# CESSProject/DeOSS

Measured on AMD Instinct MI355X. Metric: device-resident GiB/s hashed to Merkle root; 1/2/4/8 MI355X scaling, higher is better.
Workload: dtype u32; 1 GPU; BASELINE configs[1]: 1 object of 8 GiB (8589934592 B) in 1 chunk-range shard(s) of 8 GiB, chunk 33554432 B (256 leaves); object_bytes=8589934592, chunk=33554432, leaves=256, parallelism=single GPU

## Files before the change

deoss_amd/csrc/merkle_kernels.hpp:

```cpp
#pragma once
#include "sha256_gfx950.hpp"

namespace dm {

constexpr int kBlock = 256;
constexpr int kLeafFuseMax = 8;
constexpr int kReduceTile = 512;

struct LeafArgs {
    const uint8_t* base;
    uint64_t pitch;
    uint64_t leaf_len;
    uint64_t last_len;
    const uint64_t* addrs;
    const uint64_t* lens;
    uint64_t nleaves;
    uint64_t byte_off;
    uint64_t byte_end;
    uint32_t* state;
    uint8_t* digests;
    uint8_t* level_out;
    uint32_t fuse_levels;
};

__device__ __forceinline__ void load_digest(const uint8_t* p, uint32_t (&v)[8]) {
    const uint4* q = reinterpret_cast<const uint4*>(p);
    uint4 x = q[0], y = q[1];
    v[0] = bswap32(x.x); v[1] = bswap32(x.y); v[2] = bswap32(x.z); v[3] = bswap32(x.w);
    v[4] = bswap32(y.x); v[5] = bswap32(y.y); v[6] = bswap32(y.z); v[7] = bswap32(y.w);
}

__device__ __forceinline__ void store_digest(uint8_t* p, const uint32_t (&v)[8]) {
    uint4* q = reinterpret_cast<uint4*>(p);
    q[0] = make_uint4(bswap32(v[0]), bswap32(v[1]), bswap32(v[2]), bswap32(v[3]));
    q[1] = make_uint4(bswap32(v[4]), bswap32(v[5]), bswap32(v[6]), bswap32(v[7]));
}


typedef uint32_t u32x4_t __attribute__((ext_vector_type(4)));
typedef __attribute__((address_space(1))) const u32x4_t global_u32x4;

typedef __attribute__((address_space(1))) const uint8_t global_u8;
typedef __attribute__((address_space(1))) const uint32_t global_u32;

struct Blk { u32x4_t q0, q1, q2, q3; };
__device__ __forceinline__ const global_u8* gbytes(const uint8_t* p) { return (const global_u8*)p; }

template <bool ALIGNED>
__device__ __forceinline__ Blk load_block(const uint8_t* p) {
    Blk b;
    if constexpr (ALIGNED) {
        const global_u32x4* q = (const global_u32x4*)(p);
        b.q0 = q[0]; b.q1 = q[1]; b.q2 = q[2]; b.q3 = q[3];
    } else {
        uint8_t t[64];
        const global_u8* g = gbytes(p);
#pragma unroll
        for (int k = 0; k < 64; k++) t[k] = g[k];
        __builtin_memcpy(&b, t, 64);
    }
    return b;
}

__device__ __forceinline__ void block_words(const Blk& b, uint32_t (&w)[16]) {
    w[0] = bswap32(b.q0.x);  w[1] = bswap32(b.q0.y);  w[2] = bswap32(b.q0.z);  w[3] = bswap32(b.q0.w);
    w[4] = bswap32(b.q1.x);  w[5] = bswap32(b.q1.y);  w[6] = bswap32(b.q1.z);  w[7] = bswap32(b.q1.w);
    w[8] = bswap32(b.q2.x);  w[9] = bswap32(b.q2.y);  w[10] = bswap32(b.q2.z); w[11] = bswap32(b.q2.w);
    w[12] = bswap32(b.q3.x); w[13] = bswap32(b.q3.y); w[14] = bswap32(b.q3.z); w[15] = bswap32(b.q3.w);
}

#ifndef DM_K1_LINES
#define DM_K1_LINES 1
#endif
template <bool ALIGNED>
__device__ __forceinline__ void absorb_blocks(uint32_t (&st)[8], const uint8_t* p, uint64_t nb) {
    if (nb == 0) return;
    if constexpr (ALIGNED && DM_K1_LINES) {
        const uint64_t last = nb - 1;
        Blk c0 = load_block<true>(p), c1 = load_block<true>(p + 64 * (last < 1 ? last : 1));
        for (uint64_t b = 0; b < nb; b += 2) {
            const uint64_t b2 = b + 2 < last ? b + 2 : last, b3 = b + 3 < last ? b + 3 : last;
            const Blk n0 = load_block<true>(p + 64 * b2), n1 = load_block<true>(p + 64 * b3);
            __builtin_amdgcn_sched_barrier(0);
            uint32_t w[16];
            block_words(c0, w);
            compress(st, w);
            if (b + 1 < nb) {
                block_words(c1, w);
                compress(st, w);
            }
            c0 = n0;
            c1 = n1;
        }
        return;
    }
    Blk cur = load_block<ALIGNED>(p);
    for (uint64_t b = 0; b < nb; b++) {
        uint32_t w[16];
        block_words(cur, w);
        if (b + 1 < nb) cur = load_block<ALIGNED>(p + 64 * (b + 1));
        compress(st, w);
    }
}

template <bool ALIGNED>
__device__ __forceinline__ void absorb_tail(uint32_t (&st)[8], const uint8_t* p, uint32_t r, uint64_t len) {
    uint32_t w[16];
#pragma unroll
    for (int k = 0; k < 16; k++) {
        uint32_t v = 0;
        if ((uint32_t)(4 * k + 4) <= r) {
            if constexpr (ALIGNED) {
                v = bswap32(*(const global_u32*)(p + 4 * k));
            } else {
                const global_u8* g = gbytes(p);
                v = ((uint32_t)g[4 * k] << 24) | ((uint32_t)g[4 * k + 1] << 16) |
                    ((uint32_t)g[4 * k + 2] << 8) | (uint32_t)g[4 * k + 3];
            }
        } else if ((uint32_t)(4 * k) <= r) {
#pragma unroll
            for (int j = 0; j < 4; j++) {
                uint32_t idx = 4 * k + j;
                uint32_t byte = idx < r ? (uint32_t)gbytes(p)[idx] : (idx == r ? 0x80u : 0u);
                v |= byte << (24 - 8 * j);
            }
        }
        w[k] = v;
    }
    const uint64_t bits = len * 8;
    if (r <= 55) {
        w[14] = (uint32_t)(bits >> 32);
        w[15] = (uint32_t)bits;
        compress(st, w);
    } else {
        compress(st, w);
#pragma unroll
        for (int k = 0; k < 14; k++) w[k] = 0;
        w[14] = (uint32_t)(bits >> 32);
        w[15] = (uint32_t)bits;
        compress(st, w);
    }
}

__device__ __forceinline__ uint32_t lds_reduce(uint32_t (*a)[8], uint32_t (*b)[8], uint32_t cnt,
                                               uint32_t levels, uint32_t (**res)[8]) {
    const uint32_t t = threadIdx.x;
    for (uint32_t l = 0; l < levels; l++) {
        const uint32_t next = (cnt + 1) >> 1;
        if (t < next) {
            uint32_t L[8], R[8], o[8];
            const uint32_t ri = (2 * t + 1 < cnt) ? 2 * t + 1 : cnt - 1;
#pragma unroll
            for (int k = 0; k < 8; k++) { L[k] = a[2 * t][k]; R[k] = a[ri][k]; }
            node_hash(L, R, o);
#pragma unroll
            for (int k = 0; k < 8; k++) b[t][k] = o[k];
        }
        __syncthreads();
        uint32_t (*tmp)[8] = a; a = b; b = tmp;
        cnt = next;
    }
    *res = a;
    return cnt;
}

struct LeafView {
    const uint8_t* p;
    uint64_t len;
    uint64_t have;
    uint64_t nb;
    bool fin;
    bool active;
};

template <bool TABLE>
__device__ __forceinline__ LeafView leaf_view(const LeafArgs& a, uint64_t i) {
    LeafView v{};
    v.active = i < a.nleaves;
    if (!v.active) {
        v.p = a.base;
        return v;
    }
    if constexpr (TABLE) {
        v.p = reinterpret_cast<const uint8_t*>(a.addrs[i]);
        v.len = a.lens[i];
    } else {
        v.p = a.base + i * a.pitch;
        v.len = (i + 1 == a.nleaves) ? a.last_len : a.leaf_len;
    }
    const uint64_t b0 = a.byte_off;
    const uint64_t end = v.len < a.byte_end ? v.len : a.byte_end;
    v.have = end > b0 ? end - b0 : 0;
    v.fin = (b0 < v.len && v.len <= a.byte_end) || (v.len == 0 && b0 == 0);
    v.nb = v.have / 64;
    return v;
}

__device__ __forceinline__ void load_or_init_state(const LeafArgs& a, uint64_t i, uint32_t (&st)[8]) {
    if (a.state != nullptr && a.byte_off != 0) {
#pragma unroll
        for (int k = 0; k < 8; k++) st[k] = a.state[i * 8 + k];
    } else {
        init_state(st);
    }
}

template <bool ALIGNED>
__device__ __forceinline__ void leaf_epilogue(const LeafArgs& a, uint64_t i, const LeafView& v, uint32_t (&st)[8]) {
    if (v.fin) {
        absorb_tail<ALIGNED>(st, v.p + 64 * v.nb, (uint32_t)(v.have - 64 * v.nb), v.len);
        if (a.digests != nullptr) store_digest(a.digests + 32 * i, st);
    } else if (a.state != nullptr && v.have != 0) {
#pragma unroll
        for (int k = 0; k < 8; k++) a.state[i * 8 + k] = st[k];
    }
}

__device__ __forceinline__ uint64_t wave_min_u64(uint64_t x) {
#pragma unroll
    for (int o = 32; o > 0; o >>= 1) {
        const uint64_t y = __shfl_xor(x, o, 64);
        x = y < x ? y : x;
    }
    return x;
}

__device__ __forceinline__ uint64_t uniform_u64(uint64_t x) {
    return ((uint64_t)__builtin_amdgcn_readfirstlane((uint32_t)(x >> 32)) << 32) |
           __builtin_amdgcn_readfirstlane((uint32_t)x);
}

__device__ __forceinline__ uint64_t wave_max_u64(uint64_t x) {
#pragma unroll
    for (int o = 32; o > 0; o >>= 1) {
        const uint64_t y = __shfl_xor(x, o, 64);
        x = y > x ? y : x;
    }
    return x;
}

template <bool TABLE, bool ALIGNED>
__global__ __launch_bounds__(kBlock) void leaf_kernel(LeafArgs a) {
    __shared__ uint32_t lds_a[kBlock][8];
    __shared__ uint32_t lds_b[kBlock / 2][8];
    const uint64_t i = (uint64_t)blockIdx.x * kBlock + threadIdx.x;
    const LeafView v = leaf_view<TABLE>(a, i);
    const bool active = v.active;
    uint32_t st[8];
    if (active) {
        load_or_init_state(a, i, st);
        absorb_blocks<ALIGNED>(st, v.p, v.nb);
        leaf_epilogue<ALIGNED>(a, i, v, st);
    }
    if (a.fuse_levels == 0) return;
    const uint64_t first = (uint64_t)blockIdx.x * kBlock;
    const uint32_t cnt = (uint32_t)((a.nleaves - first) < kBlock ? (a.nleaves - first) : kBlock);
    if (active) {
#pragma unroll
        for (int k = 0; k < 8; k++) lds_a[threadIdx.x][k] = st[k];
    }
    __syncthreads();
    uint32_t (*res)[8];
    const uint32_t out_cnt = lds_reduce(lds_a, lds_b, cnt, a.fuse_levels, &res);
    if (threadIdx.x < out_cnt) {
        uint32_t v[8];
#pragma unroll
        for (int k = 0; k < 8; k++) v[k] = res[threadIdx.x][k];
        const uint64_t o = (uint64_t)blockIdx.x * (kBlock >> a.fuse_levels) + threadIdx.x;
        store_digest(a.level_out + 32 * o, v);
    }
}

constexpr int kLatLeaves = 64;
constexpr int kLatThreads = 128;
constexpr int kLatRing = 2;
constexpr int kLatFuseMax = 6;

__device__ __forceinline__ void rounds_from_kw(uint32_t (&st)[8], const uint4 (*kw)[kLatLeaves], uint32_t lane) {
    uint32_t a = st[0], b = st[1], c = st[2], d = st[3], e = st[4], f = st[5], g = st[6], h = st[7];
    uint4 x = kw[0][lane], y = kw[1][lane];
#pragma unroll
    for (int q = 0; q < 16; q += 2) {
        uint4 nx = x, ny = y;
        if (q + 2 < 16) {
            nx = kw[q + 2][lane];
            ny = kw[q + 3][lane];
        }
        DM_SHA_ROUND(a, b, c, d, e, f, g, h, x.x);
        DM_SHA_ROUND(h, a, b, c, d, e, f, g, x.y);
        DM_SHA_ROUND(g, h, a, b, c, d, e, f, x.z);
        DM_SHA_ROUND(f, g, h, a, b, c, d, e, x.w);
        DM_SHA_ROUND(e, f, g, h, a, b, c, d, y.x);
        DM_SHA_ROUND(d, e, f, g, h, a, b, c, y.y);
        DM_SHA_ROUND(c, d, e, f, g, h, a, b, y.z);
        DM_SHA_ROUND(b, c, d, e, f, g, h, a, y.w);
        x = nx;
        y = ny;
    }
    st[0] += a; st[1] += b; st[2] += c; st[3] += d;
    st[4] += e; st[5] += f; st[6] += g; st[7] += h;
}

__device__ __forceinline__ void schedule_to_lds(uint32_t (&w)[16], uint4 (*kw)[kLatLeaves], uint32_t lane) {
// ... 88 lines not shown
        X7 = t_ + dpp_swap_pairs(y_);                                                  \
    } while (0)

__device__ __forceinline__ void pair_rounds_from_kw(uint32_t (&x)[4], const uint4 (*kw)[kLatLeaves], uint32_t lane,
                                                    uint32_t sh1, uint32_t sh2, uint32_t sh3, uint32_t msk,
                                                    bool lane_b) {
    uint32_t x4 = x[0], x5 = x[1], x6 = x[2], x7 = x[3];
    uint4 q = kw[0][lane];
#pragma unroll
    for (int g = 0; g < 16; g++) {
        uint4 nq = q;
        if (g + 1 < 16) nq = kw[g + 1][lane];
        DM_PAIR_ROUND(x4, x5, x6, x7, q.x);
        DM_PAIR_ROUND(x7, x4, x5, x6, q.y);
        DM_PAIR_ROUND(x6, x7, x4, x5, q.z);
        DM_PAIR_ROUND(x5, x6, x7, x4, q.w);
        q = nq;
    }
    x[0] += x4; x[1] += x5; x[2] += x6; x[3] += x7;
}

template <bool TABLE, bool ALIGNED>
__global__ __launch_bounds__(kLatThreads) void leaf_kernel_pair(LeafArgs a) {
    __shared__ uint4 ring[kLatRing][16][kLatLeaves];
    __shared__ uint32_t lds_a[kPairLeaves][8];
    __shared__ uint32_t lds_b[kPairLeaves / 2][8];
    const uint32_t lane = threadIdx.x & (kLatLeaves - 1);
    const bool producer = __builtin_amdgcn_readfirstlane(threadIdx.x) < kLatLeaves;
    const bool lane_b = (lane & 1) != 0;
    const uint32_t c = lane >> 1;
    const uint64_t first = (uint64_t)blockIdx.x * kPairLeaves;
    const uint64_t i = first + c;
    const LeafView v = leaf_view<TABLE>(a, i);
    const uint64_t NB = wave_max_u64(v.nb);
    if (producer) {
        Blk cur;
        if (v.nb > 0 && !lane_b) cur = load_block<ALIGNED>(v.p);
        for (uint64_t b = 0; b < NB; b++) {
            if (b < v.nb) {
                uint32_t w[16];
                block_words(cur, w);
                if (b + 1 < v.nb && !lane_b) cur = load_block<ALIGNED>(v.p + 64 * (b + 1));
                uint4 (*kw)[kLatLeaves] = ring[b % kLatRing];
#pragma unroll
                for (int q = 0; q < 16; q++) {
                    uint32_t u[4];
#pragma unroll
                    for (int j = 0; j < 4; j++) {
                        const int t = 4 * q + j;
                        uint32_t wt;
                        if (t < 16) {
                            wt = w[t];
                        } else {
                            wt = ssig1(w[(t - 2) & 15]) + w[(t - 7) & 15] + ssig0(w[(t - 15) & 15]) + w[t & 15];
                            w[t & 15] = wt;
                        }
                        u[j] = lane_b ? 0u : kSha256K[t] + wt;
                    }
                    kw[q][lane] = make_uint4(u[0], u[1], u[2], u[3]);
                }
            }
            __syncthreads();
        }
        __syncthreads();
    } else {
        const uint32_t sh1 = lane_b ? 2 : 6, sh2 = lane_b ? 13 : 11, sh3 = lane_b ? 22 : 25;
        const uint32_t msk = lane_b ? 0u : ~0u;
        uint32_t st0[8];
        if (v.active) load_or_init_state(a, i, st0);
        else init_state(st0);
        uint32_t x[4];
#pragma unroll
        for (int k = 0; k < 4; k++) x[k] = lane_b ? st0[k] : st0[4 + k];
        __syncthreads();
        for (uint64_t b = 0; b < NB; b++) {
            if (b < v.nb) pair_rounds_from_kw(x, ring[b % kLatRing], lane, sh1, sh2, sh3, msk, lane_b);
            __syncthreads();
        }
        uint32_t st[8];
#pragma unroll
        for (int k = 0; k < 4; k++) {
            const uint32_t other = dpp_swap_pairs(x[k]);
            st[k] = lane_b ? x[k] : other;
            st[4 + k] = lane_b ? other : x[k];
        }
        if (v.active && !lane_b) {
            leaf_epilogue<ALIGNED>(a, i, v, st);
#pragma unroll
            for (int k = 0; k < 8; k++) lds_a[c][k] = st[k];
        }
    }
    if (a.fuse_levels == 0) return;
    __syncthreads();
    const uint32_t cnt = (uint32_t)((a.nleaves - first) < kPairLeaves ? (a.nleaves - first) : kPairLeaves);
    uint32_t (*res)[8];
    const uint32_t out_cnt = lds_reduce(lds_a, lds_b, cnt, a.fuse_levels, &res);
    if (threadIdx.x < out_cnt) {
        uint32_t o8[8];
#pragma unroll
        for (int k = 0; k < 8; k++) o8[k] = res[threadIdx.x][k];
        const uint64_t o = (uint64_t)blockIdx.x * (kPairLeaves >> a.fuse_levels) + threadIdx.x;
        store_digest(a.level_out + 32 * o, o8);
    }
}

constexpr int kQuadLeaves = 8;
constexpr int kQuadBlocks = 8;
constexpr int kQuadFuseMax = 3;
constexpr int kQuadRow = kQuadLeaves;
constexpr size_t kQuadLdsBytes = sizeof(uint4) * kLatRing * 16 * kQuadBlocks * kQuadRow + 4 * 8 * kQuadLeaves +
                                 4 * 8 * (kQuadLeaves / 2);
static_assert(4 * kQuadLdsBytes <= (160u << 10), "four compact K1Q workgroups must fit a CU's LDS");

#define DM_QS_HEAD(X4, X5, X6)                                                                   \
    "v_alignbit_b32 %[r], %[" X4 "], %[" X4 "], %[sh]\n\t"                                      \
    "v_bitop3_b32 %[f], %[" X4 "], %[" X5 "], %[msk] bitop3:0x1e\n\t"                          \
    "v_bitop3_b32 %[f], %[f], %[" X6 "], %[" X5 "] bitop3:0xca\n\t"                             \
    "v_xor_b32_dpp %[s], %[r], %[r] quad_perm:[1,2,0,3] row_mask:0xf bank_mask:0xf\n\t"
#define DM_QS_SIGMA "v_xor_b32_dpp %[s], %[r], %[s] quad_perm:[2,0,1,3] row_mask:0xf bank_mask:0xf\n\t"
#define DM_QS_STEP_Q(X4, X5, X6, X7, H, HN, VN, QP)                                             \
    DM_QS_HEAD(X4, X5, X6)                                                                       \
    "v_sub_u32_dpp %[" X6 "], %[" VN "], %[" X6 "] quad_perm:" QP " row_mask:0xf bank_mask:0x3\n\t" \
    DM_QS_SIGMA                                                                                  \
    "v_sub_u32_dpp %[" HN "], %[" X4 "], %[" X6 "] row_ror:8 row_mask:0xf bank_mask:0xf\n\t"    \
    "v_add3_u32 %[" X7 "], %[s], %[f], %[" H "]\n\t"
#define DM_QS_STEP(X4, X5, X6, X7, H, HN, VN) DM_QS_STEP_Q(X4, X5, X6, X7, H, HN, VN, "[0,1,2,3]")
#define DM_QS_STEP_A(X4, X5, X6, X7, H, HN)                                                     \
    DM_QS_HEAD(X4, X5, X6)                                                                       \
    DM_QS_SIGMA                                                                                  \
    "v_sub_u32_dpp %[" HN "], %[" X4 "], %[" X6 "] row_ror:8 row_mask:0xf bank_mask:0xf\n\t"    \
    "v_add3_u32 %[" X7 "], %[s], %[f], %[" H "]\n\t"
#define DM_QS_STEP_END(X4, X5, X6, X7, H)                                                       \
    DM_QS_HEAD(X4, X5, X6)                                                                       \
    DM_QS_SIGMA                                                                                  \
    "v_add3_u32 %[" X7 "], %[s], %[f], %[" H "]\n\t"
#define DM_QS_STEPS4V(V0, V1, V2, V3)                                                          \
    DM_QS_STEP("a", "b", "c", "d", "h", "g", V0) DM_QS_STEP("d", "a", "b", "c", "g", "h", V1)   \
    DM_QS_STEP("c", "d", "a", "b", "h", "g", V2) DM_QS_STEP("b", "c", "d", "a", "g", "h", V3)
#define DM_QS_ALIGN_MIS ".p2align 3\n\t.if %[mis]\n\ts_nop 0\n\t.endif\n\t"
#define DM_QS_PROLOGUE(V) DM_QS_PROLOGUE_AT(V, DM_QS_ALIGN_MIS, "[0,1,2,3]")
#define DM_QS_PROLOGUE_AT(V, ALIGN, QP)                                                           \
    "s_nop 1\n\t" ALIGN                                                                          \
    "v_sub_u32_dpp %[d], %[" V "], %[d] quad_perm:" QP " row_mask:0xf bank_mask:0x3\n\t"         \
    "v_sub_u32_dpp %[h], %[b], %[d] row_ror:8 row_mask:0xf bank_mask:0xf\n\t"
#define DM_QS_RESTORE_A(P, X) "v_mov_b32_dpp %[" P "], %[" X "] quad_perm:[0,1,2,3] row_mask:0xf bank_mask:0xc\n\t"
#define DM_QS_GROUP0(V0, V1, V2, V3)                                                             \
    DM_QS_STEP("a", "b", "c", "d", "h", "g", V0) DM_QS_RESTORE_A("d", "x3")                      \
    DM_QS_STEP("d", "a", "b", "c", "g", "h", V1) DM_QS_RESTORE_A("c", "x2")                      \
    DM_QS_STEP("c", "d", "a", "b", "h", "g", V2) DM_QS_STEP("b", "c", "d", "a", "g", "h", V3)
#define DM_QS_FF(X, P, BANKS) "v_add_u32_dpp %[" X "], %[" P "], %[" X "] quad_perm:[0,1,2,3] row_mask:0xf bank_mask:" BANKS "\n\t"
#define DM_QS_TAIL(V0, V1, V2)                                                                   \
    DM_QS_STEP("a", "b", "c", "d", "h", "g", V0) DM_QS_STEP("d", "a", "b", "c", "g", "h", V1)   \
    DM_QS_STEP("c", "d", "a", "b", "h", "g", V2) DM_QS_STEP_A("b", "c", "d", "a", "g", "h")      \
    DM_QS_FF("x3", "d", "0x3") DM_QS_FF("x2", "c", "0x3") DM_QS_FF("x1", "b", "0x3")             \
    DM_QS_FF("x0", "a", "0x3")                                                                   \
    DM_QS_STEP_A("a", "b", "c", "d", "h", "g") DM_QS_STEP_END("d", "a", "b", "c", "g")           \
    DM_QS_FF("x0", "a", "0xc") DM_QS_FF("x1", "b", "0xc") DM_QS_FF("x3", "d", "0xc")             \
    DM_QS_FF("x2", "c", "0xc")
#define DM_QS_STEPS4Q(V0, Q0, V1, Q1, V2, Q2, V3, Q3)                                          \
    DM_QS_STEP_Q("a", "b", "c", "d", "h", "g", V0, Q0) DM_QS_STEP_Q("d", "a", "b", "c", "g", "h", V1, Q1) \
    DM_QS_STEP_Q("c", "d", "a", "b", "h", "g", V2, Q2) DM_QS_STEP_Q("b", "c", "d", "a", "g", "h", V3, Q3)
#define DM_QS_GROUP0Q(V0, Q0, V1, Q1, V2, Q2, V3, Q3)                                          \
    DM_QS_STEP_Q("a", "b", "c", "d", "h", "g", V0, Q0) DM_QS_RESTORE_A("d", "x3")              \
    DM_QS_STEP_Q("d", "a", "b", "c", "g", "h", V1, Q1) DM_QS_RESTORE_A("c", "x2")              \
    DM_QS_STEP_Q("c", "d", "a", "b", "h", "g", V2, Q2) DM_QS_STEP_Q("b", "c", "d", "a", "g", "h", V3, Q3)
#define DM_QS_TAILQ(V0, Q0, V1, Q1, V2, Q2)                                                     \
    DM_QS_STEP_Q("a", "b", "c", "d", "h", "g", V0, Q0) DM_QS_STEP_Q("d", "a", "b", "c", "g", "h", V1, Q1) \
    DM_QS_STEP_Q("c", "d", "a", "b", "h", "g", V2, Q2) DM_QS_STEP_A("b", "c", "d", "a", "g", "h") \
    DM_QS_FF("x3", "d", "0x3") DM_QS_FF("x2", "c", "0x3") DM_QS_FF("x1", "b", "0x3")             \
    DM_QS_FF("x0", "a", "0x3")                                                                   \
    DM_QS_STEP_A("a", "b", "c", "d", "h", "g") DM_QS_STEP_END("d", "a", "b", "c", "g")           \
    DM_QS_FF("x0", "a", "0xc") DM_QS_FF("x1", "b", "0xc") DM_QS_FF("x3", "d", "0xc")             \
    DM_QS_FF("x2", "c", "0xc")
#define DM_QS_OUT                                                                                \
    : [a] "+v"(p0), [b] "+v"(p1), [c] "+v"(p2), [d] "+v"(p3), [h] "+v"(h), [g] "+v"(g),           \
      [x0] "+v"(x[0]), [x1] "+v"(x[1]), [x2] "+v"(x[2]), [x3] "+v"(x[3]), [r] "=&v"(r_),          \
      [f] "=&v"(f_), [s] "=&v"(s_)
#define DM_QS_OPS DM_QS_OUT : [mis] "i"(MIS ? 1 : 0), [sh] "v"(sh.x), [msk] "v"(msk), [v0] "v"(v0), [v1] "v"(v1), [v2] "v"(v2), [v3] "v"(v3)

template <bool MIS, class KW>
__device__ __forceinline__ void quad_block_skewed(uint32_t (&x)[4], KW kw, uint3 sh, uint32_t msk) {
    uint32_t p0 = x[0], p1 = x[1], p2 = x[2], p3 = x[3], h = 0, g = 0, r_, f_, s_;
    uint4 q = kw(0), nq = kw(1);
    {
        const uint32_t v0 = q.x, v1 = 0, v2 = 0, v3 = 0;
        asm volatile(DM_QS_PROLOGUE("v0") DM_QS_OPS);
    }
#pragma unroll
    for (int grp = 0; grp < 16; grp++) {
        const uint4 nnq = grp + 2 < 16 ? kw(grp + 2) : nq;
        const uint32_t v0 = q.y, v1 = q.z, v2 = q.w, v3 = nq.x;
        if (grp == 0) {
            asm volatile(DM_QS_ALIGN_MIS DM_QS_GROUP0("v0", "v1", "v2", "v3") DM_QS_OPS);
        } else if (grp < 15) {
            asm volatile(DM_QS_ALIGN_MIS DM_QS_STEPS4V("v0", "v1", "v2", "v3") DM_QS_OPS);
        } else {
            asm volatile(DM_QS_ALIGN_MIS DM_QS_TAIL("v0", "v1", "v2") DM_QS_OPS);
        }
        q = nq;
        nq = nnq;
    }
}

constexpr int kLgkmWait0 = 0xC07F;

#define DM_QS_HNB(HN, A, B, BANKS) "v_sub_u32_dpp %[" HN "], %[" A "], %[" B "] row_ror:8 row_mask:0xf bank_mask:" BANKS "\n\t"
#define DM_QS_ADDB(D, A, B, BANKS) "v_add_u32_dpp %[" D "], %[" A "], %[" B "] quad_perm:[0,1,2,3] row_mask:0xf bank_mask:" BANKS "\n\t"
#define DM_QS_MOVB(D, S, BANKS) "v_mov_b32_dpp %[" D "], %[" S "] quad_perm:[0,1,2,3] row_mask:0xf bank_mask:" BANKS "\n\t"
#define DM_QS_KWN(X6, S, N) "v_sub_u32_dpp %[" X6 "], %[" N "], %[" S "] quad_perm:[0,0,0,0] row_mask:0xf bank_mask:0x3\n\t"
#define DM_QS_ADD3(X7, H) "v_add3_u32 %[" X7 "], %[s], %[f], %[" H "]\n\t"
#define DM_QS_LINKQ(V0, Q0, V1, Q1, V2, Q2, N0, N1, N2)                                          \
    DM_QS_STEP_Q("a", "b", "c", "d", "h", "g", V0, Q0) DM_QS_STEP_Q("d", "a", "b", "c", "g", "h", V1, Q1) \
    DM_QS_STEP_Q("c", "d", "a", "b", "h", "g", V2, Q2)                                           \
    DM_QS_ADDB("x1", "x1", "b", "0xc") DM_QS_ADDB("x3", "x3", "d", "0x3")                        \
                                            \
    DM_QS_HEAD("b", "c", "d") DM_QS_KWN("d", "x3", N0) DM_QS_SIGMA                               \
    DM_QS_HNB("h", "x1", "d", "0x3") DM_QS_HNB("h", "b", "d", "0xc") DM_QS_ADD3("a", "g")        \
    DM_QS_ADDB("b", "x1", "b", "0x3") DM_QS_ADDB("c", "x2", "c", "0x3")                          \
    DM_QS_HNB("g", "a", "c", "0xc") DM_QS_ADDB("x0", "x0", "a", "0xc")                           \
    DM_QS_ADDB("a", "a", "x0", "0x3") DM_QS_MOVB("x2", "c", "0x3")                               \
                                                            \
    DM_QS_HEAD("a", "b", "c") DM_QS_KWN("c", "c", N1) DM_QS_SIGMA                                \
    DM_QS_HNB("g", "x0", "c", "0x3") DM_QS_ADD3("d", "h")                                        \
    DM_QS_ADDB("x3", "x3", "d", "0xc") DM_QS_MOVB("x1", "b", "0x3") DM_QS_MOVB("x0", "a", "0x3") \
                                           \
    DM_QS_HEAD("d", "a", "b") DM_QS_KWN("b", "b", N2) DM_QS_SIGMA                                \
    DM_QS_HNB("h", "x3", "b", "0x3") DM_QS_HNB("h", "d", "x1", "0xc") DM_QS_ADD3("c", "g")       \
    DM_QS_ADDB("x2", "x2", "c", "0xc") DM_QS_MOVB("a", "x0", "0xc") DM_QS_MOVB("d", "x3", "0xc") \
    DM_QS_MOVB("c", "x2", "0xc")
#define DM_QS_BODYQ                                                                              \
    DM_QS_STEPS4Q("q01", "[1,1,1,1]", "q02", "[1,1,1,1]", "q03", "[1,1,1,1]", "q00", "[2,2,2,2]") \
    DM_QS_STEPS4Q("q01", "[2,2,2,2]", "q02", "[2,2,2,2]", "q03", "[2,2,2,2]", "q00", "[3,3,3,3]") \
    DM_QS_STEPS4Q("q01", "[3,3,3,3]", "q02", "[3,3,3,3]", "q03", "[3,3,3,3]", "q10", "[0,0,0,0]") \
    DM_QS_STEPS4Q("q11", "[0,0,0,0]", "q12", "[0,0,0,0]", "q13", "[0,0,0,0]", "q10", "[1,1,1,1]") \
    DM_QS_STEPS4Q("q11", "[1,1,1,1]", "q12", "[1,1,1,1]", "q13", "[1,1,1,1]", "q10", "[2,2,2,2]") \
    DM_QS_STEPS4Q("q11", "[2,2,2,2]", "q12", "[2,2,2,2]", "q13", "[2,2,2,2]", "q10", "[3,3,3,3]") \
    DM_QS_STEPS4Q("q11", "[3,3,3,3]", "q12", "[3,3,3,3]", "q13", "[3,3,3,3]", "q20", "[0,0,0,0]") \
    DM_QS_STEPS4Q("q21", "[0,0,0,0]", "q22", "[0,0,0,0]", "q23", "[0,0,0,0]", "q20", "[1,1,1,1]") \
    DM_QS_STEPS4Q("q21", "[1,1,1,1]", "q22", "[1,1,1,1]", "q23", "[1,1,1,1]", "q20", "[2,2,2,2]") \
    DM_QS_STEPS4Q("q21", "[2,2,2,2]", "q22", "[2,2,2,2]", "q23", "[2,2,2,2]", "q20", "[3,3,3,3]") \
    DM_QS_STEPS4Q("q21", "[3,3,3,3]", "q22", "[3,3,3,3]", "q23", "[3,3,3,3]", "q30", "[0,0,0,0]") \
    DM_QS_STEPS4Q("q31", "[0,0,0,0]", "q32", "[0,0,0,0]", "q33", "[0,0,0,0]", "q30", "[1,1,1,1]") \
    DM_QS_STEPS4Q("q31", "[1,1,1,1]", "q32", "[1,1,1,1]", "q33", "[1,1,1,1]", "q30", "[2,2,2,2]") \
    DM_QS_STEPS4Q("q31", "[2,2,2,2]", "q32", "[2,2,2,2]", "q33", "[2,2,2,2]", "q30", "[3,3,3,3]")
#define DM_QS_FILLQ                                                                              \
    DM_QS_PROLOGUE_AT("q00", DM_QS_ALIGN_MIS, "[0,0,0,0]")                                       \
    DM_QS_GROUP0Q("q01", "[0,0,0,0]", "q02", "[0,0,0,0]", "q03", "[0,0,0,0]", "q00", "[1,1,1,1]")
#define DM_QS_CONTQ                                                                              \
    DM_QS_ALIGN_MIS                                                                              \
    DM_QS_STEP_Q("c", "d", "a", "b", "h", "g", "q03", "[0,0,0,0]") DM_QS_STEP_Q("b", "c", "d", "a", "g", "h", "q00", "[1,1,1,1]")
#define DM_QS_ENDLINKQ DM_QS_LINKQ("q31", "[3,3,3,3]", "q32", "[3,3,3,3]", "q33", "[3,3,3,3]", "n0", "n1", "n2")
#define DM_QS_ENDTAILQ DM_QS_TAILQ("q31", "[3,3,3,3]", "q32", "[3,3,3,3]", "q33", "[3,3,3,3]")
#define DM_QS_STATE [a] "+v"(P[0]), [b] "+v"(P[1]), [c] "+v"(P[2]), [d] "+v"(P[3]),              \
                    [x0] "+v"(x[0]), [x1] "+v"(x[1]), [x2] "+v"(x[2]), [x3] "+v"(x[3]),           \
                    [r] "=&v"(r_), [f] "=&v"(f_), [s] "=&v"(s_)
#define DM_QS_KIN [mis] "i"(MIS ? 1 : 0), [sh] "v"(sh.x), [msk] "v"(msk),                        \
                  [q00] "v"(K[0].x), [q01] "v"(K[0].y), [q02] "v"(K[0].z), [q03] "v"(K[0].w),     \
                  [q10] "v"(K[1].x), [q11] "v"(K[1].y), [q12] "v"(K[1].z), [q13] "v"(K[1].w),     \
                  [q20] "v"(K[2].x), [q21] "v"(K[2].y), [q22] "v"(K[2].z), [q23] "v"(K[2].w),     \
                  [q30] "v"(K[3].x), [q31] "v"(K[3].y), [q32] "v"(K[3].z), [q33] "v"(K[3].w)

template <bool MIS, int K8>
__device__ __forceinline__ void quad_block_regs(uint32_t (&x)[4], uint32_t (&P)[4], uint32_t& h, uint32_t& g,
                                                const uint4 (&K)[4], const uint4& N, uint3 sh, uint32_t msk) {
    uint32_t r_, f_, s_;
    if constexpr (K8 == 0) {
        asm volatile(DM_QS_FILLQ DM_QS_BODYQ DM_QS_ENDLINKQ
                     : DM_QS_STATE, [h] "=&v"(h), [g] "=&v"(g)
                     : DM_QS_KIN, [n0] "v"(N.x), [n1] "v"(N.y), [n2] "v"(N.z));
    } else if constexpr (K8 < kQuadBlocks - 1) {
        asm volatile(DM_QS_CONTQ DM_QS_BODYQ DM_QS_ENDLINKQ
                     : DM_QS_STATE, [h] "+v"(h), [g] "+v"(g)
                     : DM_QS_KIN, [n0] "v"(N.x), [n1] "v"(N.y), [n2] "v"(N.z));
    } else {
        asm volatile(DM_QS_CONTQ DM_QS_BODYQ DM_QS_ENDTAILQ
                     : DM_QS_STATE, [h] "+v"(h), [g] "+v"(g)
                     : DM_QS_KIN);
    }
}

template <int G, int ROW, bool MIS, int K8 = 0>
__device__ __forceinline__ void quad_stage_blocks(uint32_t (&x)[4], uint32_t (&P)[4], uint32_t& h, uint32_t& g,
                                                  uint4 (&S)[3][4], const uint4* kw, uint3 sh, uint32_t msk) {
    __builtin_amdgcn_s_waitcnt(kLgkmWait0);
    if constexpr (K8 + 2 < kQuadBlocks) {
#pragma unroll
        for (int t = 0; t < 4; t++) S[(K8 + 2) % 3][t] = kw[(K8 + 2) * ROW + 4 * t * G];
    }
    quad_block_regs<MIS, K8>(x, P, h, g, S[K8 % 3], S[(K8 + 1) % 3][0], sh, msk);
    if constexpr (K8 + 1 < kQuadBlocks) quad_stage_blocks<G, ROW, MIS, K8 + 1>(x, P, h, g, S, kw, sh, msk);
}
template <int G, int ROW, bool MIS>
__device__ __forceinline__ void quad_stage_regs(uint32_t (&x)[4], const uint4* kw, uint3 sh, uint32_t msk) {
    uint4 S[3][4];
    uint32_t P[4] = {x[0], x[1], x[2], x[3]}, h, g;
#pragma unroll
    for (int k = 0; k < 2; k++) {
#pragma unroll
        for (int t = 0; t < 4; t++) S[k][t] = kw[k * ROW + 4 * t * G];
    }
    quad_stage_blocks<G, ROW, MIS>(x, P, h, g, S, kw, sh, msk);
}

template <bool TABLE, bool ALIGNED, bool COMPACT>
__global__ __launch_bounds__(kLatThreads) void leaf_kernel_quad(LeafArgs a) {
    constexpr int ROW = COMPACT ? kQuadRow : kQuadLeaves;
    constexpr int G = kQuadBlocks * ROW;
    __shared__ uint4 ring[COMPACT ? 1 : 2][kLatRing][16][G];
    __shared__ uint32_t lds_a[kQuadLeaves][8];
    __shared__ uint32_t lds_b[kQuadLeaves / 2][8];
    const uint32_t lane = threadIdx.x & 63;
    const bool producer = __builtin_amdgcn_readfirstlane(threadIdx.x) < 64;
    const uint32_t c = lane >> 3;
    const uint32_t j = lane & 7;
    const uint64_t first = (uint64_t)blockIdx.x * kQuadLeaves;
    const uint64_t i = first + c;
    const LeafView v = leaf_view<TABLE>(a, i);
    const uint64_t NB = wave_max_u64(v.nb);
    const uint64_t NI = (NB + kQuadBlocks - 1) / kQuadBlocks;
    if (producer) {
        Blk cur;
        if (j < v.nb) cur = load_block<ALIGNED>(v.p + 64 * j);
        for (uint64_t it = 0; it < NI; it++) {
            const uint64_t b = it * kQuadBlocks + j;
            if (b < v.nb) {
                uint32_t w[16];
                block_words(cur, w);
                if (b + kQuadBlocks < v.nb) cur = load_block<ALIGNED>(v.p + 64 * (b + kQuadBlocks));
                uint4* kw = &ring[0][it % kLatRing][0][j * ROW + c];
#pragma unroll
                for (int q = 0; q < 16; q++) {
                    uint32_t u[4];
#pragma unroll
                    for (int k = 0; k < 4; k++) {
                        const int t = 4 * q + k;
                        uint32_t wt;
                        if (t < 16) {
                            wt = w[t];
                        } else {
                            wt = ssig1(w[(t - 2) & 15]) + w[(t - 7) & 15] + ssig0(w[(t - 15) & 15]) + w[t & 15];
                            w[t & 15] = wt;
                        }
                        u[k] = 0u - (kSha256K[t] + wt);
                    }
                    kw[q * G] = make_uint4(u[0], u[1], u[2], u[3]);
                }
            }
            __syncthreads();
        }
        __syncthreads();
    } else {
        __builtin_amdgcn_s_setprio(1);
        const uint32_t cq = 2 * (lane >> 4) + ((lane >> 2) & 1);
        const bool role_a = (lane >> 3) & 1;
        const uint32_t p = lane & 3;
        const uint64_t iq = first + cq;
        const LeafView vq = leaf_view<TABLE>(a, iq);
        const uint3 sh = make_uint3(role_a ? (p == 0 ? 2 : p == 1 ? 13 : 22) : (p == 0 ? 6 : p == 1 ? 11 : 25), 0, 0);
        const uint32_t msk = role_a ? 0u : ~0u;
        uint32_t st0[8];
        if (vq.active) load_or_init_state(a, iq, st0);
        else init_state(st0);
        uint32_t x[4];
#pragma unroll
        for (int k = 0; k < 4; k++) x[k] = role_a ? st0[(k + 2) & 3] : st0[4 + k];
        const uint4* col = &ring[0][0][0][cq];
        __syncthreads();
        uint32_t xf[4];
#pragma unroll
        for (int k = 0; k < 4; k++) xf[k] = x[k];
        const uint64_t NS = uniform_u64(NI);
        for (uint64_t it = 0; it < NS;) {
            const bool running = vq.active && vq.nb > it * kQuadBlocks;
            const uint64_t end = uniform_u64(wave_min_u64(running ? vq.nb / kQuadBlocks : NS));
            for (; it < end; it++) {
                quad_stage_regs<G, ROW, COMPACT>(x, col + (it % kLatRing) * 16 * G + p * G, sh, msk);
                __syncthreads();
            }
            if (running) {
#pragma unroll
                for (int k = 0; k < 4; k++) xf[k] = x[k];
            }
            if (it == NS) break;
            if (!__any(vq.active && vq.nb > it * kQuadBlocks && vq.nb < (it + 1) * kQuadBlocks)) continue;
            const uint4* kw = col + (it % kLatRing) * 16 * G;
            const uint64_t b0 = it * kQuadBlocks;
            for (uint32_t k = 0; k < kQuadBlocks; k++) {
                const uint4* kb = kw + k * ROW;
                if (b0 + k < vq.nb)
                    quad_block_skewed<COMPACT>(x, [kb](int g) { return kb[g * G]; }, sh, msk);
            }
            if (vq.nb > b0) {
#pragma unroll
                for (int k = 0; k < 4; k++) xf[k] = x[k];
            }
            __syncthreads();
            it++;
        }
        uint32_t st[8];
#pragma unroll
        for (int k = 0; k < 4; k++) {
            st[k] = __shfl(xf[(k + 2) & 3], (int)(lane + 8), 64);
            st[4 + k] = xf[k];
        }
        if (vq.active && !role_a && p == 0) {
            leaf_epilogue<ALIGNED>(a, iq, vq, st);
#pragma unroll
            for (int k = 0; k < 8; k++) lds_a[cq][k] = st[k];
        }
    }
    if (a.fuse_levels == 0) return;
    __syncthreads();
    const uint32_t cnt = (uint32_t)((a.nleaves - first) < kQuadLeaves ? (a.nleaves - first) : kQuadLeaves);
    uint32_t (*res)[8];
    const uint32_t out_cnt = lds_reduce(lds_a, lds_b, cnt, a.fuse_levels, &res);
    if (threadIdx.x < out_cnt) {
        uint32_t o8[8];
#pragma unroll
        for (int k = 0; k < 8; k++) o8[k] = res[threadIdx.x][k];
        const uint64_t o = (uint64_t)blockIdx.x * (kQuadLeaves >> a.fuse_levels) + threadIdx.x;
        store_digest(a.level_out + 32 * o, o8);
    }
}

__global__ __launch_bounds__(kLatThreads) void quad_shape_primer(int x) {
    extern __shared__ uint4 dyn[];
    if (x == 12345) dyn[threadIdx.x] = make_uint4(1, 1, 1, 1);
}

__global__ __launch_bounds__(kBlock) void reduce_kernel(const uint8_t* in, uint64_t m, uint32_t levels,
                                                         uint8_t* out) {
    __shared__ uint32_t lds_a[kBlock][8];
    __shared__ uint32_t lds_b[kBlock / 2][8];
    const uint64_t base = (uint64_t)blockIdx.x * kReduceTile;
    const uint32_t cnt = (uint32_t)((m - base) < kReduceTile ? (m - base) : kReduceTile);
    const uint32_t t = threadIdx.x;
    const uint32_t next = (cnt + 1) >> 1;
    if (t < next) {
        uint32_t L[8], R[8], o[8];
        const uint32_t ri = (2 * t + 1 < cnt) ? 2 * t + 1 : cnt - 1;
        load_digest(in + 32 * (base + 2 * t), L);
        load_digest(in + 32 * (base + ri), R);
        node_hash(L, R, o);
#pragma unroll
        for (int k = 0; k < 8; k++) lds_a[t][k] = o[k];
    }
    __syncthreads();
    uint32_t (*res)[8];
    const uint32_t out_cnt = lds_reduce(lds_a, lds_b, next, levels - 1, &res);
    if (t < out_cnt) {
        uint32_t v[8];
#pragma unroll
        for (int k = 0; k < 8; k++) v[k] = res[t][k];
        store_digest(out + 32 * ((uint64_t)blockIdx.x * (kReduceTile >> levels) + t), v);
    }
}

__global__ __launch_bounds__(kBlock) void batch_root_kernel(const uint8_t* leaves, const uint64_t* leaf_first,
                                                             const uint32_t* obj_ids, uint8_t* roots) {
    __shared__ uint32_t lds_a[kBlock][8];
    __shared__ uint32_t lds_b[kBlock / 2][8];
    const uint32_t o = obj_ids[blockIdx.x];
    const uint64_t base = leaf_first[o];
    const uint32_t cnt = (uint32_t)(leaf_first[o + 1] - base);
    const uint32_t t = threadIdx.x;
    const uint32_t next = (cnt + 1) >> 1;
    if (t < next) {
        uint32_t L[8], R[8], h[8];
        const uint32_t ri = (2 * t + 1 < cnt) ? 2 * t + 1 : cnt - 1;
        load_digest(leaves + 32 * (base + 2 * t), L);
        load_digest(leaves + 32 * (base + ri), R);
        node_hash(L, R, h);
#pragma unroll
        for (int k = 0; k < 8; k++) lds_a[t][k] = h[k];
    }
    __syncthreads();
    uint32_t levels = 0;
    for (uint32_t c = next; c > 1; c = (c + 1) >> 1) levels++;
    uint32_t (*res)[8];
    lds_reduce(lds_a, lds_b, next, levels, &res);
    if (t == 0) {
        uint32_t v[8];
#pragma unroll
        for (int k = 0; k < 8; k++) v[k] = res[0][k];
        store_digest(roots + 32 * (uint64_t)o, v);
    }
}

__device__ __forceinline__ uint64_t splitmix64(uint64_t z) {
    z += 0x9e3779b97f4a7c15ULL;
    z = (z ^ (z >> 30)) * 0xbf58476d1ce4e5b9ULL;
    z = (z ^ (z >> 27)) * 0x94d049bb133111ebULL;
    return z ^ (z >> 31);
}

__global__ __launch_bounds__(kBlock) void fill_splitmix_kernel(uint64_t* dst, uint64_t word0, uint64_t nwords,
                                                                uint64_t seed) {
    const uint64_t stride = (uint64_t)gridDim.x * kBlock * 2;
    for (uint64_t j = ((uint64_t)blockIdx.x * kBlock + threadIdx.x) * 2; j < nwords; j += stride) {
        if (j + 1 < nwords) {
            ulonglong2 v = make_ulonglong2(splitmix64(seed ^ (word0 + j)), splitmix64(seed ^ (word0 + j + 1)));
            *reinterpret_cast<ulonglong2*>(dst + j) = v;
        } else {
            dst[j] = splitmix64(seed ^ (word0 + j));
        }
    }
}

constexpr int kProbeLoads = 16;
__global__ __launch_bounds__(kBlock) void read_probe_kernel(const uint8_t* p, uint64_t n16, uint64_t* out) {
    const u32x4_t* g = reinterpret_cast<const u32x4_t*>(p);
    const uint64_t per = (n16 + gridDim.x - 1) / gridDim.x;
    const uint64_t lo = (uint64_t)blockIdx.x * per, hi = lo + per < n16 ? lo + per : n16;
    u32x4_t acc[kProbeLoads];
#pragma unroll
    for (int u = 0; u < kProbeLoads; u++) acc[u] = u32x4_t{0u, 0u, 0u, 0u};
    uint64_t i = lo + threadIdx.x;
    for (; i + (kProbeLoads - 1) * kBlock < hi; i += kProbeLoads * kBlock) {
        u32x4_t x[kProbeLoads];
#pragma unroll
        for (int u = 0; u < kProbeLoads; u++) x[u] = __builtin_nontemporal_load(g + i + u * kBlock);
#pragma unroll
        for (int u = 0; u < kProbeLoads; u++) acc[u] ^= x[u];
    }
    for (; i < hi; i += kBlock) acc[0] ^= g[i];
#pragma unroll
    for (int u = 1; u < kProbeLoads; u++) acc[0] ^= acc[u];
    uint64_t v = (((uint64_t)acc[0].y << 32) | acc[0].x) ^ (((uint64_t)acc[0].w << 32) | acc[0].z);
    for (int m = 32; m >= 1; m >>= 1) v ^= __shfl_xor(v, m, 64);
    __shared__ uint64_t part[kBlock / 64];
    if ((threadIdx.x & 63) == 0) part[threadIdx.x >> 6] = v;
    __syncthreads();
    if (threadIdx.x == 0) {
        uint64_t t = 0;
        for (int w = 0; w < kBlock / 64; w++) t ^= part[w];
        atomicXor(reinterpret_cast<unsigned long long*>(out), (unsigned long long)t);
    }
}

}
```

deoss_amd/isa.py:

```python
from __future__ import annotations

import json
import os
import re
import subprocess
import tempfile

HERE = os.path.dirname(os.path.abspath(__file__))
COUNTS = os.path.join(HERE, "isa_counts.json")
SLOT_WEIGHTS = {"v_alignbit_b32": 2.0, "v_add3_u32": 2.0, "v_xad_u32": 2.0}
KERNELS = {
    "wide": ("_ZN2dm11leaf_kernelILb0ELb1EEEvNS_8LeafArgsE", (1, 0)),
    "latency": ("_ZN2dm15leaf_kernel_latILb0ELb1EEEvNS_8LeafArgsE", (1, 1)),
    "pair": ("_ZN2dm16leaf_kernel_pairILb0ELb1EEEvNS_8LeafArgsE", (2, 2)),
    "quad": ("_ZN2dm16leaf_kernel_quadILb0ELb1ELb0EEEvNS_8LeafArgsE", (8, 1)),
}
K1_SYMBOL = KERNELS["wide"][0]


def _function_body(asm: str, sym: str) -> list:
    lines = asm.splitlines()
    start = None
    for i, ln in enumerate(lines):
        if ln.startswith(sym + ":"):
            start = i
            break
    if start is None:
        raise ValueError(f"{sym} not found in assembly")
    body = []
    for ln in lines[start + 1:]:
        if ln.startswith(".Lfunc_end") or re.match(r"^\s*\.size\s+" + re.escape(sym), ln):
            break
        body.append(ln)
    return body


def _loops(body: list):
    labels, insts = {}, []
    skip = []
    for ln in body:
        s = ln.strip()
        m = re.match(r"^\.if\s+(\S+)", s)
        if m:
            skip.append(m.group(1) == "0")
            continue
        if s.startswith(".endif"):
            if skip:
                skip.pop()
            continue
        if any(skip):
            continue
        m = re.match(r"^(\.LBB[0-9_]+):", s)
        if m:
            labels[m.group(1)] = len(insts)
            continue
        if not s or s.startswith(";") or s.startswith("."):
            continue
        insts.append(s.split(";")[0].strip())
    for i, ins in enumerate(insts):
        m = re.match(r"^s_c?branch\w*\s+(\.LBB[0-9_]+)", ins)
        if m and m.group(1) in labels and labels[m.group(1)] <= i:
            yield insts[labels[m.group(1)]:i + 1]


def _summary(loop: list, per: int) -> dict:
    valu = [x for x in loop if x.startswith("v_")]
    hist = {}
    for x in valu:
        op = x.split()[0]
        hist[op] = hist.get(op, 0) + 1
    slots = sum(SLOT_WEIGHTS.get(x.split()[0], 1.0) for x in valu)
    return {"valu": round(len(valu) / per, 1), "valu_slots": round(slots / per, 1),
            "blocks_per_iteration": per, "salu": sum(1 for x in loop if x.startswith("s_")),
            "lds": sum(1 for x in loop if x.startswith("ds_")),
            "vmem": sum(1 for x in loop if x.startswith(("global_", "buffer_", "flat_"))),
            "total": len(loop), "valu_histogram": dict(sorted(hist.items(), key=lambda kv: -kv[1]))}


def _smallest(loops, pred):
    best = None
    for lp in loops:
        if pred(lp) and (best is None or len(lp) < len(best)):
            best = lp
    return best


def analyse(asm: str, sym: str = K1_SYMBOL) -> dict:
    loops = [l for l in _loops(_function_body(asm, sym))
             if sum(x.startswith("global_load_dwordx4") for x in l) >= 4]
    if not loops:
        raise ValueError("no block loop found")
    lp = max(loops, key=len)
    loads = sum(x.startswith("global_load_dwordx4") for x in lp)
    return _summary(lp, max(1, loads // 4))


def analyse_split(asm: str, sym: str) -> dict:
    loops = list(_loops(_function_body(asm, sym)))
    stage = _smallest(loops, lambda l: sum(x.startswith("v_add3_u32") for x in l) >= 8 * 64 + 2
                      and sum(x.startswith("ds_read_b128") for x in l) >= 32)
    if stage is not None:
        prod = _smallest(loops, lambda l: sum(x.startswith("ds_write_b128") for x in l) >= 16)
        if prod is None:
            raise ValueError(f"{sym}: producer loop not found")
        return {"consumer": _summary(stage, 8), "producer": _summary(prod, 1)}
    cons = _smallest(loops, lambda l: sum(x.startswith("ds_read_b128") for x in l) >= 16)
    prod = _smallest(loops, lambda l: sum(x.startswith("ds_write_b128") for x in l) >= 16)
    if cons is None or prod is None:
        raise ValueError(f"{sym}: consumer/producer loop not found")
    return {"consumer": _summary(cons, 1), "producer": _summary(prod, 1)}


def generate(write: bool = True) -> dict:
    from . import build as b
    with tempfile.TemporaryDirectory() as td:
        out = os.path.join(td, "lib.so")
        cmd = b.hipcc_cmd(out, extra=("-save-temps",))
        subprocess.run(cmd, check=True, cwd=td, capture_output=True)
        asm_files = [f for f in os.listdir(td) if f.endswith(".s") and "gfx950" in f]
        asm = open(os.path.join(td, asm_files[0])).read()
    res = {}
    for name, (sym, lanes) in KERNELS.items():
        if name == "wide":
            d = analyse(asm, sym)
            d["lane_slots_per_leaf_block"] = d["valu_slots"]
        else:
            d = analyse_split(asm, sym)
            d["lane_slots_per_leaf_block"] = (d["consumer"]["valu_slots"] * lanes[0] +
                                              d["producer"]["valu_slots"] * lanes[1])
            d["consumer_valu_per_block"] = d["consumer"]["valu"]
        d["kernel"] = sym
        d["lanes_per_leaf_block"] = {"consumer": lanes[0], "producer": lanes[1]}
        res[name] = d
    res["per"] = "one 64-byte block of one leaf"
    if write:
        with open(COUNTS, "w") as f:
            json.dump(res, f, indent=1)
    return res


def kernel_counts(kind: str = "wide"):
    try:
        with open(COUNTS) as f:
            d = json.load(f)[kind]
    except (OSError, KeyError, ValueError):
        return None, None
    ops = d["valu"] if kind == "wide" else d["consumer_valu_per_block"]
    return ops, d["lane_slots_per_leaf_block"]


def valu_per_block():
    return kernel_counts("wide")


def chain_instructions_per_block(kind: str):
    try:
        with open(COUNTS) as f:
            d = json.load(f)[kind]
    except (OSError, KeyError, ValueError):
        return None
    w = d if kind == "wide" else d.get("consumer", {})
    if "total" not in w or not w.get("blocks_per_iteration"):
        return None
    return w["total"] / w["blocks_per_iteration"]


if __name__ == "__main__":
    print(json.dumps(generate(), indent=1))
```

Before: 16.72 GiB/s.

## Deepen wide quad ring to three stages with cross-stage register prefetch

For the non-compact quad leaf kernel, the producer now runs up to two stages ahead using a three-deep LDS ring. The consumer uses a new cross-stage run loop that prefetches the next stage's message words into a rotating register set before the barrier, so the barrier no longer drains the pipeline. The aim is to hide producer latency and LDS-read stalls at stage boundaries while keeping two workgroups per CU. The cost is more complex slot bookkeeping and a higher risk of ring-indexing bugs on partial-leaf tails.

```diff
diff --git a/deoss_amd/csrc/merkle_kernels.hpp b/deoss_amd/csrc/merkle_kernels.hpp
--- a/deoss_amd/csrc/merkle_kernels.hpp
+++ b/deoss_amd/csrc/merkle_kernels.hpp
@@ -1,4 +1,5 @@
 #pragma once
+#include "quad_ring.hpp"
 #include "sha256_gfx950.hpp"
 
 namespace dm {
@@ -693,13 +694,97 @@
     quad_stage_blocks<G, ROW, MIS>(x, P, h, g, S, kw, sh, msk);
 }
 
+constexpr int kQuadWideRing = quad_ring::kWideDepth;
+constexpr int kQuadSets = quad_ring::kSets;
+template <int G, int ROW, int K8, bool FILL, bool TAIL, bool LOAD>
+__device__ __forceinline__ void quad_xstage_block(uint32_t (&x)[4], uint32_t (&P)[4], uint32_t& h, uint32_t& g,
+                                                  uint4 (&S)[kQuadSets][4], const uint4* src, uint3 sh, uint32_t msk) {
+    static_assert((LOAD || !quad_ring::block_prefetches(K8, true)) && (!TAIL || !quad_ring::block_links(K8, true)) &&
+                      !(FILL && TAIL) && quad_ring::prefetch_of(K8).block == (K8 + quad_ring::kAhead) % kQuadBlocks,
+                  "only the last stage of a run skips a load or drains: quad_ring.hpp");
+    __builtin_amdgcn_s_waitcnt(kLgkmWait0);
+    if constexpr (LOAD) {
+        constexpr quad_ring::BlockRef pf = quad_ring::prefetch_of(K8);
+#pragma unroll
+        for (int t = 0; t < 4; t++) S[quad_ring::set_of(K8 + quad_ring::kAhead)][t] = src[pf.block * ROW + 4 * t * G];
+    }
+    quad_block_regs<false, FILL ? 0 : TAIL ? kQuadBlocks - 1 : 1>(x, P, h, g, S[quad_ring::set_of(K8)],
+                                                                 S[quad_ring::set_of(K8 + 1)][0], sh, msk);
+}
+template <int G, int ROW>
+__device__ __forceinline__ uint32_t quad_run_xstage(uint32_t (&x)[4], const uint4* colp, uint32_t slot, uint64_t n,
+                                                    uint3 sh, uint32_t msk) {
+    uint4 S[kQuadSets][4];
+    uint32_t P[4] = {x[0], x[1], x[2], x[3]}, h, g;
+    const uint4* cur = colp + slot * 16 * G;
+#pragma unroll
+    for (int k = 0; k < quad_ring::kAhead; k++) {
+#pragma unroll
+        for (int t = 0; t < 4; t++) S[k][t] = cur[k * ROW + 4 * t * G];
+    }
+    quad_xstage_block<G, ROW, 0, true, false, true>(x, P, h, g, S, cur, sh, msk);
+    for (uint64_t s = 1; s < n; s++) {
+        slot = quad_ring::next_slot(slot, kQuadWideRing);
+        const uint4* nxt = colp + slot * 16 * G;
+        quad_xstage_block<G, ROW, 1, false, false, true>(x, P, h, g, S, cur, sh, msk);
+        quad_xstage_block<G, ROW, 2, false, false, true>(x, P, h, g, S, cur, sh, msk);
+        quad_xstage_block<G, ROW, 3, false, false, true>(x, P, h, g, S, cur, sh, msk);
+        quad_xstage_block<G, ROW, 4, false, false, true>(x, P, h, g, S, cur, sh, msk);
+        quad_xstage_block<G, ROW, 5, false, false, true>(x, P, h, g, S, cur, sh, msk);
+        quad_xstage_block<G, ROW, 6, false, false, true>(x, P, h, g, S, nxt, sh, msk);
+        quad_xstage_block<G, ROW, 7, false, false, true>(x, P, h, g, S, nxt, sh, msk);
+        __syncthreads();
+        quad_xstage_block<G, ROW, 0, false, false, true>(x, P, h, g, S, nxt, sh, msk);
+        cur = nxt;
+    }
+    quad_xstage_block<G, ROW, 1, false, false, true>(x, P, h, g, S, cur, sh, msk);
+    quad_xstage_block<G, ROW, 2, false, false, true>(x, P, h, g, S, cur, sh, msk);
+    quad_xstage_block<G, ROW, 3, false, false, true>(x, P, h, g, S, cur, sh, msk);
+    quad_xstage_block<G, ROW, 4, false, false, true>(x, P, h, g, S, cur, sh, msk);
+    quad_xstage_block<G, ROW, 5, false, false, true>(x, P, h, g, S, cur, sh, msk);
+    quad_xstage_block<G, ROW, 6, false, false, false>(x, P, h, g, S, cur, sh, msk);
+    quad_xstage_block<G, ROW, 7, false, true, false>(x, P, h, g, S, cur, sh, msk);
+    __syncthreads();
+    return quad_ring::next_slot(slot, kQuadWideRing);
+}
+
+template <bool ALIGNED, int G>
+__device__ __forceinline__ void quad_produce_block(const LeafView& v, Blk& cur, uint64_t b, uint4* kw) {
+    if (b >= v.nb) return;
+    uint32_t w[16];
+    block_words(cur, w);
+    if (b + kQuadBlocks < v.nb) cur = load_block<ALIGNED>(v.p + 64 * (b + kQuadBlocks));
+#pragma unroll
+    for (int q = 0; q < 16; q++) {
+        uint32_t u[4];
+#pragma unroll
+        for (int k = 0; k < 4; k++) {
+            const int t = 4 * q + k;
+            uint32_t wt;
+            if (t < 16) {
+                wt = w[t];
+            } else {
+                wt = ssig1(w[(t - 2) & 15]) + w[(t - 7) & 15] + ssig0(w[(t - 15) & 15]) + w[t & 15];
+                w[t & 15] = wt;
+            }
+            u[k] = 0u - (kSha256K[t] + wt);
+        }
+        kw[q * G] = make_uint4(u[0], u[1], u[2], u[3]);
+    }
+}
+
 template <bool TABLE, bool ALIGNED, bool COMPACT>
 __global__ __launch_bounds__(kLatThreads) void leaf_kernel_quad(LeafArgs a) {
     constexpr int ROW = COMPACT ? kQuadRow : kQuadLeaves;
     constexpr int G = kQuadBlocks * ROW;
+    constexpr int DEPTH = COMPACT ? kLatRing : kQuadWideRing;
     __shared__ uint4 ring[COMPACT ? 1 : 2][kLatRing][16][G];
     __shared__ uint32_t lds_a[kQuadLeaves][8];
     __shared__ uint32_t lds_b[kQuadLeaves / 2][8];
+    static_assert(DEPTH * sizeof(ring[0][0]) <= sizeof(ring), "the ring's stages must fit its LDS");
+    static_assert(COMPACT || (3 * sizeof(ring) > (160u << 10) && sizeof(ring) <= (64u << 10) &&
+                              2 * (sizeof(ring) + sizeof(lds_a) + sizeof(lds_b)) <= (160u << 10)),
+                  "the wide K1Q must stay at exactly two workgroups per CU (160 KiB of LDS)");
     const uint32_t lane = threadIdx.x & 63;
     const bool producer = __builtin_amdgcn_readfirstlane(threadIdx.x) < 64;
     const uint32_t c = lane >> 3;
@@ -712,34 +797,50 @@
     if (producer) {
         Blk cur;
         if (j < v.nb) cur = load_block<ALIGNED>(v.p + 64 * j);
-        for (uint64_t it = 0; it < NI; it++) {
-            const uint64_t b = it * kQuadBlocks + j;
-            if (b < v.nb) {
-                uint32_t w[16];
-                block_words(cur, w);
-                if (b + kQuadBlocks < v.nb) cur = load_block<ALIGNED>(v.p + 64 * (b + kQuadBlocks));
-                uint4* kw = &ring[0][it % kLatRing][0][j * ROW + c];
-#pragma unroll
-                for (int q = 0; q < 16; q++) {
-                    uint32_t u[4];
-#pragma unroll
-                    for (int k = 0; k < 4; k++) {
-                        const int t = 4 * q + k;
-                        uint32_t wt;
-                        if (t < 16) {
-                            wt = w[t];
-                        } else {
-                            wt = ssig1(w[(t - 2) & 15]) + w[(t - 7) & 15] + ssig0(w[(t - 15) & 15]) + w[t & 15];
-                            w[t & 15] = wt;
+        if constexpr (!COMPACT) {
+            uint4* const kw0 = &ring[0][0][0][j * ROW + c];
+            uint32_t slot = 0;
+            for (uint64_t s = 0; s < quad_ring::stages_before_first_barrier(DEPTH); s++) {
+                if (s < NI) quad_produce_block<ALIGNED, G>(v, cur, s * kQuadBlocks + j, kw0 + slot * 16 * G);
+                slot = quad_ring::next_slot(slot, DEPTH);
+            }
+            __syncthreads();
+            for (uint64_t it = 0; it < NI; it++) {
+                const uint64_t s = quad_ring::stage_written_after_barrier(it, DEPTH);
+                if (s < NI) quad_produce_block<ALIGNED, G>(v, cur, s * kQuadBlocks + j, kw0 + slot * 16 * G);
+                slot = quad_ring::next_slot(slot, DEPTH);
+                __syncthreads();
+            }
+        } else {
+            for (uint64_t it = 0; it < NI; it++) {
+                const uint64_t b = it * kQuadBlocks + j;
+                if (b < v.nb) {
+                    uint32_t w[16];
+                    block_words(cur, w);
+                    if (b + kQuadBlocks < v.nb) cur = load_block<ALIGNED>(v.p + 64 * (b + kQuadBlocks));
+                    uint4* kw = &ring[0][it % kLatRing][0][j * ROW + c];
+#pragma unroll
+                    for (int q = 0; q < 16; q++) {
+                        uint32_t u[4];
+#pragma unroll
+                        for (int k = 0; k < 4; k++) {
+                            const int t = 4 * q + k;
+                            uint32_t wt;
+                            if (t < 16) {
+                                wt = w[t];
+                            } else {
+                                wt = ssig1(w[(t - 2) & 15]) + w[(t - 7) & 15] + ssig0(w[(t - 15) & 15]) + w[t & 15];
+                                w[t & 15] = wt;
+                            }
+                            u[k] = 0u - (kSha256K[t] + wt);
                         }
-                        u[k] = 0u - (kSha256K[t] + wt);
+                        kw[q * G] = make_uint4(u[0], u[1], u[2], u[3]);
                     }
-                    kw[q * G] = make_uint4(u[0], u[1], u[2], u[3]);
                 }
+                __syncthreads();
             }
             __syncthreads();
         }
-        __syncthreads();
     } else {
         __builtin_amdgcn_s_setprio(1);
         const uint32_t cq = 2 * (lane >> 4) + ((lane >> 2) & 1);
@@ -761,20 +862,30 @@
 #pragma unroll
         for (int k = 0; k < 4; k++) xf[k] = x[k];
         const uint64_t NS = uniform_u64(NI);
+        uint32_t wslot = 0;
         for (uint64_t it = 0; it < NS;) {
-            const bool running = vq.active && vq.nb > it * kQuadBlocks;
-            const uint64_t end = uniform_u64(wave_min_u64(running ? vq.nb / kQuadBlocks : NS));
-            for (; it < end; it++) {
-                quad_stage_regs<G, ROW, COMPACT>(x, col + (it % kLatRing) * 16 * G + p * G, sh, msk);
-                __syncthreads();
+            const bool running = COMPACT ? vq.active && vq.nb > it * kQuadBlocks
+                                         : quad_ring::leaf_running(vq.active, vq.nb, it);
+            const uint64_t end = uniform_u64(wave_min_u64(COMPACT ? (running ? vq.nb / kQuadBlocks : NS)
+                                                                  : quad_ring::leaf_run_end(running, vq.nb, NS)));
+            if constexpr (COMPACT) {
+                for (; it < end; it++) {
+                    quad_stage_regs<G, ROW, COMPACT>(x, col + (it % kLatRing) * 16 * G + p * G, sh, msk);
+                    __syncthreads();
+                }
+            } else if (it < end) {
+                wslot = quad_run_xstage<G, ROW>(x, col + p * G, wslot, end - it, sh, msk);
+                it = end;
             }
             if (running) {
 #pragma unroll
                 for (int k = 0; k < 4; k++) xf[k] = x[k];
             }
             if (it == NS) break;
-            if (!__any(vq.active && vq.nb > it * kQuadBlocks && vq.nb < (it + 1) * kQuadBlocks)) continue;
-            const uint4* kw = col + (it % kLatRing) * 16 * G;
+            if (!__any(COMPACT ? vq.active && vq.nb > it * kQuadBlocks && vq.nb < (it + 1) * kQuadBlocks
+                               : quad_ring::leaf_ends_inside(vq.active, vq.nb, it)))
+                continue;
+            const uint4* kw = col + (COMPACT ? (uint32_t)(it % kLatRing) : wslot) * 16 * G;
             const uint64_t b0 = it * kQuadBlocks;
             for (uint32_t k = 0; k < kQuadBlocks; k++) {
                 const uint4* kb = kw + k * ROW;
@@ -787,6 +898,7 @@
             }
             __syncthreads();
             it++;
+            wslot = quad_ring::next_slot(wslot, DEPTH);
         }
         uint32_t st[8];
 #pragma unroll
diff --git a/deoss_amd/csrc/quad_ring.hpp b/deoss_amd/csrc/quad_ring.hpp
--- /dev/null
+++ b/deoss_amd/csrc/quad_ring.hpp
@@ -0,0 +1,42 @@
+#pragma once
+#include <cstdint>
+
+namespace dm {
+namespace quad_ring {
+
+constexpr int kBlocks = 8;
+constexpr int kWideDepth = 3;
+constexpr int kAhead = 2;
+constexpr int kSets = 4;
+static_assert(kBlocks % kSets == 0 && kSets > kAhead, "a block's register set must not depend on the stage");
+
+constexpr uint64_t stages(uint64_t max_blocks) { return (max_blocks + kBlocks - 1) / kBlocks; }
+constexpr uint64_t barriers(uint64_t ni) { return ni + 1; }
+constexpr uint32_t slot_of(uint64_t stage, int depth) { return (uint32_t)(stage % (uint64_t)depth); }
+constexpr uint32_t next_slot(uint32_t slot, int depth) { return slot + 1 == (uint32_t)depth ? 0 : slot + 1; }
+
+constexpr uint64_t stages_before_first_barrier(int depth) { return (uint64_t)depth - 1; }
+constexpr uint64_t stage_written_after_barrier(uint64_t it, int depth) { return it + (uint64_t)depth - 1; }
+constexpr uint64_t complete_after_barrier(uint64_t b, int depth) { return b + (uint64_t)depth - 1; }
+
+constexpr bool leaf_running(bool active, uint64_t nb, uint64_t it) { return active && nb > it * kBlocks; }
+constexpr uint64_t leaf_run_end(bool running, uint64_t nb, uint64_t ns) { return running ? nb / kBlocks : ns; }
+constexpr bool leaf_ends_inside(bool active, uint64_t nb, uint64_t it) {
+    return active && nb > it * kBlocks && nb < (it + 1) * kBlocks;
+}
+
+struct BlockRef {
+    uint32_t dstage;
+    uint32_t block;
+};
+constexpr BlockRef prefetch_of(uint32_t k) { return BlockRef{(k + kAhead) / kBlocks, (k + kAhead) % kBlocks}; }
+constexpr uint32_t set_of(uint32_t k) { return k % kSets; }
+constexpr bool block_prefetches(uint32_t k, bool last_stage_of_run) {
+    return !(last_stage_of_run && k + kAhead >= (uint32_t)kBlocks);
+}
+constexpr bool block_links(uint32_t k, bool last_stage_of_run) {
+    return !(last_stage_of_run && k + 1 == (uint32_t)kBlocks);
+}
+
+}
+}
diff --git a/deoss_amd/isa.py b/deoss_amd/isa.py
--- a/deoss_amd/isa.py
+++ b/deoss_amd/isa.py
@@ -97,7 +97,7 @@
 
 def analyse_split(asm: str, sym: str) -> dict:
     loops = list(_loops(_function_body(asm, sym)))
-    stage = _smallest(loops, lambda l: sum(x.startswith("v_add3_u32") for x in l) >= 8 * 64 + 2
+    stage = _smallest(loops, lambda l: sum(x.startswith("v_add3_u32") for x in l) >= 8 * 64
                       and sum(x.startswith("ds_read_b128") for x in l) >= 32)
     if stage is not None:
         prod = _smallest(loops, lambda l: sum(x.startswith("ds_write_b128") for x in l) >= 16)
```

Result: faster. 16.89 GiB/s (median of 6 runs) (+1.1%).
